# mlvlab/UP-NeRF

Measured on AMD Instinct MI355X. Metric: training rays/sec, higher is better.
Workload: dtype f32 (f16x3 emulated: 3 fp16 MFMAs per product, fp32 accumulate); 1 GPU; BASELINE.json configs[1]: Brandenburg Gate shape, 4096 rays/GPU/step, 64 coarse + 128 fine samples, two 8x256 fields + candidate/colour heads + TransientNet + appearance/candidate embeddings (763 images), pose optimisation ON, full step incl. both Adam updates; rays_per_gpu=4096, n_images=763, N_samples=64, N_importance=128, parallelism=dp1, field=f16x3

## Files before the change

include/upnerf_hip.h:

```cpp
#ifndef UPNERF_HIP_H
#define UPNERF_HIP_H

#include <stdint.h>

#ifdef __cplusplus
extern "C" {
#endif

#define UPNERF_ABI_VERSION 11
#define UPNERF_EINVAL (-1)
#define UPNERF_EUNSUP (-2)

#ifndef UPNERF_TILE_ROWS
#define UPNERF_TILE_ROWS 64
#endif
#define UPNERF_X0 64
#define UPNERF_AUXK 80
#define UPNERF_CK 16
#define UPNERF_MAX_D 8

int upnerf_abi_version(void);

int upnerf_pose_rays_fwd(int R, const float* se3, const float* c2w, const float* dirs,
                         float* rays_o, float* rays_d, void* stream);
// ... 246 lines not shown
int upnerf_transient_fwd(const upnerf_transient_args* a, void* stream);
int upnerf_transient_bwd(const upnerf_transient_args* a, const upnerf_transient_grads* g, void* stream);

enum {
  UPNERF_WG_F32 = 0,
  UPNERF_WG_F16_TILE,
  UPNERF_WG_F16_FRAG,
  UPNERF_WG_F24,
  UPNERF_WG_PLANES
};
typedef struct {
  const void* p;
  const void* lo;
  const int32_t* exp;
  int32_t ld, kind;
} upnerf_wgrad_operand;

typedef struct {
  const float* slabs; const float* bslabs;
  float* dW; float* db;
  int32_t N, K, TN, TK, nsplit, ldo, rblocks;
  int32_t n2;
  float* dW2; float* db2;
  int32_t ldo2, pad;
  const float* vslabs; float* dv; float* dbv;
} upnerf_wgrad_pending;

typedef struct {
  int32_t M, N, K;
  int32_t planes;
  upnerf_wgrad_operand A, B;
  const int32_t* expo_a; const int32_t* expo_b;
  float* dW; float* db;
  int32_t ldo;
  int32_t n2;
  float* dW2; float* db2;
  int32_t ldo2, nsplit;
  const float* v; float* dv; float* dbv;
  float* slabs;
} upnerf_wgrad_desc;
long long upnerf_wgrad16_scratch(const upnerf_wgrad_desc* d);
int upnerf_wgrad16(const upnerf_wgrad_desc* d, upnerf_wgrad_pending* pending, void* stream);
int upnerf_wgrad_finish(upnerf_wgrad_pending* pending, void* stream);

int upnerf_vec_wgrad(int M, const float* v, int ldv, int nvec, const float* X, int ldx, int K,
                     float* dw , float* dbv , float* scratch, int nsplit, void* stream);

int upnerf_vec_wgrad_frag16(int M, const float* v, int ldv, int nvec, const uint16_t* X16, const int32_t* xexp, int K, float* dw,
                            float* dbv, float* scratch, int nsplit, void* stream);

int upnerf_ray_sum(int R, int S, const float* X, int C, float* out, void* stream);
int upnerf_ray_geom_bwd(int R, int S, const float* dxyz, const float* z, float* d_o, float* d_d, void* stream);

typedef struct {
  int32_t R, h, C;
  const int64_t* idx;
  const float* all_ray_infos;
  const float* all_directions;
  const float* all_rgbs;
  const float* all_pxl_coords;
  const float* all_inv_depths;
  const float* feat_maps;
  const float* poses;
  float* ray_infos;
  float* directions;
  int64_t* img_idx;
  float* c2w;
  float* rgbs;
  float* feats;
  float* inv_depths;
} upnerf_gather_rays_args;
int upnerf_gather_rays(const upnerf_gather_rays_args* a, void* stream);

int upnerf_embed_bwd(int R, int N, int dim, const int64_t* idx, const float* g, float* out, void* stream);
#define UPNERF_MAX_EMBED_GROUPS 8
typedef struct {
  const float* g;
  float* out;
  int32_t dim;
} upnerf_embed_group;
int upnerf_embed_bwd_grouped(int R, int N, const int64_t* idx, const upnerf_embed_group* groups, int ngroups, void* stream);
typedef struct {
  const float* table;
  float* rows;
  int32_t dim;
} upnerf_embed_rows_group;
int upnerf_embed_fwd_grouped(int R, int N, const int64_t* idx, const upnerf_embed_rows_group* groups, int ngroups, void* stream);


int upnerf_linear(int M, int N, int K, const float* A, int lda, const float* B, int ldb,
                  const float* bias, float* C, int ldc, int act, void* stream);
int upnerf_matvec(int M, int K, const float* A, int lda, const float* x, const float* add, float* y, int trans, void* stream);
int upnerf_zero(float* p, long long n, void* stream);
#define UPNERF_MAX_ADD_PAIRS 8
typedef struct upnerf_add_pair {
  const float* a;
  const float* b;
  float* out;
  int32_t n;
} upnerf_add_pair;
int upnerf_add_pairs(const upnerf_add_pair* pairs, int npairs, void* stream);
int upnerf_matvec_rank1(int M, int K, const float* A, int lda, const float* x, float* y, float* R, int ldr, const float* v,
                        void* stream);

typedef struct {
  int32_t R, F, fine, has_tw;
// ... 797 lines not shown
```

upnerf_amd/_lib.py:

```python
from __future__ import annotations

import ctypes as C
import os

import torch

from .pass_plan import (AUXK, CK, RR_PART_STRIDE, TILE_PART_STRIDE, WG_F16_FRAG, WG_F16_TILE, WG_F24, WG_F32,
                        WG_PLANES, X0)

_HERE = os.path.dirname(os.path.abspath(__file__))
LIB_PATH = os.environ.get("UPNERF_LIB") or os.path.join(_HERE, "libupnerf_hip.so")
MAX_D = 8

_fp = C.c_void_p


class Layout(C.Structure):
    _fields_ = [("W", C.c_int32), ("D", C.c_int32), ("skip", C.c_int32),
                ("w", C.c_int32 * MAX_D), ("b", C.c_int32 * MAX_D),
                ("we", C.c_int32), ("be", C.c_int32), ("wsig", C.c_int32), ("bsig", C.c_int32),
                ("wc1", C.c_int32), ("bc1", C.c_int32), ("wc2", C.c_int32), ("bc2", C.c_int32),
                ("wcsig", C.c_int32), ("bcsig", C.c_int32), ("wr1", C.c_int32), ("br1", C.c_int32),
                ("wr2", C.c_int32), ("br2", C.c_int32), ("total", C.c_int32),
                ("t_w", C.c_int32 * MAX_D), ("t_skipx", C.c_int32), ("t_we", C.c_int32), ("t_head", C.c_int32),
# ... 93 lines not shown

class WgradPending(C.Structure):
    _fields_ = [("slabs", _fp), ("bslabs", _fp), ("dW", _fp), ("db", _fp), ("N", C.c_int32), ("K", C.c_int32), ("TN", C.c_int32),
                ("TK", C.c_int32), ("nsplit", C.c_int32), ("ldo", C.c_int32), ("rblocks", C.c_int32), ("n2", C.c_int32),
                ("dW2", _fp), ("db2", _fp), ("ldo2", C.c_int32), ("pad", C.c_int32), ("vslabs", _fp), ("dv", _fp), ("dbv", _fp)]


class WgradOperand(C.Structure):
    _fields_ = [("p", _fp), ("lo", _fp), ("exp", _fp), ("ld", C.c_int32), ("kind", C.c_int32)]


class WgradDesc(C.Structure):
    _fields_ = [("M", C.c_int32), ("N", C.c_int32), ("K", C.c_int32), ("planes", C.c_int32), ("A", WgradOperand), ("B", WgradOperand),
                ("expo_a", _fp), ("expo_b", _fp), ("dW", _fp), ("db", _fp), ("ldo", C.c_int32), ("n2", C.c_int32), ("dW2", _fp),
                ("db2", _fp), ("ldo2", C.c_int32), ("nsplit", C.c_int32), ("v", _fp), ("dv", _fp), ("dbv", _fp), ("slabs", _fp)]


class WgradGroup(C.Structure):
    _fields_ = [("A", _fp), ("B", _fp), ("dW", _fp), ("db", _fp), ("M", C.c_int32), ("N", C.c_int32), ("K", C.c_int32),
                ("lda", C.c_int32), ("ldb", C.c_int32), ("ldo", C.c_int32)]


MAX_WGRAD_GROUPS = 32


class EmbedGroup(C.Structure):
    _fields_ = [("g", _fp), ("out", _fp), ("dim", C.c_int32)]


class EmbedRowsGroup(C.Structure):
    _fields_ = [("table", _fp), ("rows", _fp), ("dim", C.c_int32)]


MAX_EMBED_GROUPS = 8


class GatherRaysArgs(C.Structure):
    _fields_ = [("R", C.c_int32), ("h", C.c_int32), ("C", C.c_int32), ("idx", _fp),
                ("all_ray_infos", _fp), ("all_directions", _fp), ("all_rgbs", _fp), ("all_pxl_coords", _fp),
                ("all_inv_depths", _fp), ("feat_maps", _fp), ("poses", _fp),
                ("ray_infos", _fp), ("directions", _fp), ("img_idx", _fp), ("c2w", _fp), ("rgbs", _fp), ("feats", _fp),
                ("inv_depths", _fp)]


class Frag16Desc(C.Structure):
    _fields_ = FragDesc._fields_ + [("exp_id", C.c_int32)]


class AddPair(C.Structure):
    _fields_ = [("a", _fp), ("b", _fp), ("out", _fp), ("n", C.c_int32)]


MAX_ADD_PAIRS = 8


class SsimArgs(C.Structure):
    _fields_ = [("N", C.c_int32), ("C", C.c_int32), ("H", C.c_int32), ("W", C.c_int32), ("pred", _fp), ("gt", _fp),
                ("pred_stride", C.c_int64 * 4), ("gt_stride", C.c_int64 * 4), ("ssim", _fp), ("map", _fp)]


class Conv2dArgs(C.Structure):
    _fields_ = [("N", C.c_int32), ("C_in", C.c_int32), ("H", C.c_int32), ("W", C.c_int32), ("C_out", C.c_int32),
                ("k", C.c_int32), ("stride", C.c_int32), ("pad", C.c_int32), ("relu", C.c_int32), ("scale_in", C.c_int32),
                ("x", _fp), ("x_stride", C.c_int64 * 4), ("w", _fp), ("bias", _fp), ("y", _fp)]


class Maxpool2dArgs(C.Structure):
    _fields_ = [("N", C.c_int32), ("C", C.c_int32), ("H", C.c_int32), ("W", C.c_int32), ("x", _fp), ("y", _fp)]


class LpipsDistArgs(C.Structure):
    _fields_ = [("N", C.c_int32), ("C", C.c_int32), ("H", C.c_int32), ("W", C.c_int32), ("accumulate", C.c_int32),
                ("reserved_", C.c_int32), ("feat", _fp), ("w", _fp), ("out", _fp)]


class LpipsScratchArgs(C.Structure):
    _fields_ = [("N", C.c_int32), ("H", C.c_int32), ("W", C.c_int32), ("reserved_", C.c_int32),
                ("act0_elems", C.c_int64), ("act1_elems", C.c_int64), ("part_elems", C.c_int64)]


class VitPatchesArgs(C.Structure):
    _fields_ = [("H", C.c_int32), ("W", C.c_int32), ("stride", C.c_int32), ("u8", C.c_int32), ("image", _fp),
                ("mean", C.c_float * 3), ("std", C.c_float * 3), ("rows", _fp)]


class VitAttentionArgs(C.Structure):
    _fields_ = [("N", C.c_int32), ("heads", C.c_int32), ("head_dim", C.c_int32), ("reserved_", C.c_int32),
                ("q", _fp), ("k", _fp), ("v", _fp), ("ldq", C.c_int64), ("ldk", C.c_int64), ("ldv", C.c_int64),
                ("scale", C.c_float), ("reserved2_", C.c_float), ("out", _fp), ("ldo", C.c_int64)]


class PcaFitArgs(C.Structure):
    _fields_ = [("T", C.c_int32), ("D", C.c_int32), ("x", _fp), ("ldx", C.c_int64), ("mean", _fp), ("gram", _fp)]


class Conv3x3Args(C.Structure):
    _fields_ = [("H", C.c_int32), ("W", C.c_int32), ("C_in", C.c_int32), ("C_out", C.c_int32), ("stride", C.c_int32),
                ("pre_relu", C.c_int32), ("relu", C.c_int32), ("reserved_", C.c_int32), ("x", _fp), ("ldx", C.c_int64), ("w", _fp),
                ("bias", _fp), ("res", _fp), ("ldr", C.c_int64), ("y", _fp), ("ldy", C.c_int64)]


class Upsample2xArgs(C.Structure):
    _fields_ = [("H", C.c_int32), ("W", C.c_int32), ("C", C.c_int32), ("reserved_", C.c_int32), ("x", _fp), ("ldx", C.c_int64),
                ("y", _fp), ("ldy", C.c_int64)]


# ... 284 lines not shown
    _fields_ = [("M", C.c_int32), ("reserved_", C.c_int32), ("points", _fp), ("P", _fp), ("PT", _fp), ("wk_xyz", C.c_float * 10),
                ("sigma", _fp), ("grad", _fp)]


class NormalCompositeArgs(C.Structure):
    _fields_ = [("R", C.c_int32), ("S", C.c_int32), ("grad", _fp), ("w", _fp), ("normal", _fp)]


class VizNormalsArgs(C.Structure):
    _fields_ = [("H", C.c_int32), ("W", C.c_int32), ("n", _fp), ("rot", _fp), ("rgb", _fp)]


class Rng(C.Structure):
    _fields_ = [("seed", C.c_uint64), ("step", C.c_int32), ("row0", C.c_int32), ("row_stride", C.c_int32), ("step_dev", _fp)]


_i, _f, _p = C.c_int, C.c_float, C.c_void_p
_SIGNATURES = {
    "upnerf_abi_version": [],
    "upnerf_pose_rays_fwd": [_i, _p, _p, _p, _p, _p, _p],
    "upnerf_pose_rays_bwd": [_i, _p, _p, _p, _p, _p, _p, _p],
    "upnerf_sample_coarse": [_i, _i, _p, _p, _p, _f, _i, _p, _p],
    "upnerf_uniform_keyed": [_i, _i, C.c_uint64, _i, _p, _i, _i, _i, _p, _p],
    "upnerf_sample_pdf": [_i, _i, _p, _p, _p, _i, _i, _p, _i, _p],
    "upnerf_sort_rows": [_i, _i, _p, _p],
    "upnerf_sample_coarse_keyed": [_i, _i, _p, _p, C.POINTER(Rng), _f, _i, _p, _p],
    "upnerf_resample_sort": [_i, _i, _p, _p, _i, _i, _p, _i, _p, _i, _i, _p, _i, _i, C.POINTER(Rng), _p, _p],
    "upnerf_ray_aux": [_i, _p, _p, C.POINTER(C.c_float), _p, _p, _p],
    "upnerf_field_fwd": [C.POINTER(Layout), C.POINTER(FieldFwdArgs), _p],
    "upnerf_composite_fwd": [C.POINTER(CompositeFwdArgs), _p],
    "upnerf_composite_bwd": [C.POINTER(CompositeBwdArgs), _p],
    "upnerf_field_bwd": [C.POINTER(Layout), C.POINTER(FieldBwdArgs), _p],
    "upnerf_field_fwd_f16x3": [C.POINTER(Layout), C.POINTER(FieldFwdArgs), _p],
    "upnerf_field_bwd_f16x3": [C.POINTER(Layout), C.POINTER(FieldBwdArgs), _p],
    "upnerf_frag16": [_p, _p, _p, C.POINTER(Frag16Desc), _i, C.POINTER(Frag16Desc), _i, _p, _p, _i, _i, _p, _p],
    "upnerf_wgrad": [_i, _p, _i, _i, _p, _i, _i, _p, _i, _p, _p, _i, _p],
    "upnerf_wgrad16_scratch": [C.POINTER(WgradDesc)],
    "upnerf_wgrad16": [C.POINTER(WgradDesc), C.POINTER(WgradPending), _p],
    "upnerf_wgrad_finish": [_p, _p],
    "upnerf_transient_fwd": [C.POINTER(TransientArgs), _p],
    "upnerf_transient_bwd": [C.POINTER(TransientArgs), C.POINTER(TransientGrads), _p],
    "upnerf_wgrad_grouped_scratch": [C.POINTER(WgradGroup), _i, _i],
    "upnerf_wgrad_grouped": [C.POINTER(WgradGroup), _i, _p, _i, _p],
    "upnerf_vec_wgrad": [_i, _p, _i, _i, _p, _i, _i, _p, _p, _p, _i, _p],
    "upnerf_matvec": [_i, _i, _p, _i, _p, _p, _p, _i, _p],
    "upnerf_matvec_rank1": [_i, _i, _p, _i, _p, _p, _p, _i, _p, _p],
    "upnerf_add_pairs": [C.POINTER(AddPair), _i, _p],
    "upnerf_zero": [_p, C.c_longlong, _p],
    "upnerf_vec_wgrad_frag16": [_i, _p, _i, _i, _p, _p, _i, _p, _p, _p, _i, _p],
    "upnerf_ray_sum": [_i, _i, _p, _i, _p, _p],
    "upnerf_ray_part_finish": [_i, _i, _p, _p, _p, _p],
    "upnerf_tile_part_finish": [_i, _i, _p, _p, _p, _p, _p, _p, _p, _p, _p],
    "upnerf_ray_geom_bwd": [_i, _i, _p, _p, _p, _p, _p],
    "upnerf_pack": [_p, C.POINTER(PackDesc), _i, _i, _p],
    "upnerf_gather_rays": [C.POINTER(GatherRaysArgs), _p],
    "upnerf_embed_bwd": [_i, _i, _i, _p, _p, _p, _p],
    "upnerf_embed_bwd_grouped": [_i, _i, _p, C.POINTER(EmbedGroup), _i, _p],
    "upnerf_embed_fwd_grouped": [_i, _i, _p, C.POINTER(EmbedRowsGroup), _i, _p],
    "upnerf_linear": [_i, _i, _i, _p, _i, _p, _i, _p, _p, _i, _i, _p],
    "upnerf_loss_fwd": [C.POINTER(LossArgs), _p, _p, _p, _p],
    "upnerf_loss_bwd": [C.POINTER(LossArgs), _p, C.POINTER(LossGrads), _p],
    "upnerf_frag_copy": [_p, _p, C.POINTER(FragDesc), _i, _p],
    "upnerf_adam": [C.c_int64, _p, _p, _p, _p, _f, _f, _f, _f, _f, _p, _p],
    "upnerf_adam_gather": [_p, _p, _p, _p, _i, _f, _f, _f, _f, _f, _p, _p],
    "upnerf_set_scalars": [_p, _i, C.POINTER(C.c_float), _p],
    "upnerf_scale_exponents": [_p, _i, _p, _p],
    "upnerf_ssim_scratch": [C.POINTER(SsimArgs)],
    "upnerf_ssim": [C.POINTER(SsimArgs), _p, _p],
    "upnerf_conv2d": [C.POINTER(Conv2dArgs), _p],
    "upnerf_maxpool2d": [C.POINTER(Maxpool2dArgs), _p],
    "upnerf_lpips_dist": [C.POINTER(LpipsDistArgs), _p, _p],
    "upnerf_lpips_scratch": [C.POINTER(LpipsScratchArgs)],
    "upnerf_scene_rays": [C.POINTER(SceneRaysArgs), C.POINTER(SceneImage), _p, _p],
    "upnerf_resize_scratch": [C.POINTER(ResizeArgs)],
    "upnerf_resize_linear": [C.POINTER(ResizeArgs), C.POINTER(ResizeMap), _p, _p],
    "upnerf_viz_minmax_scratch": [C.c_longlong],
    "upnerf_viz_minmax": [_p, C.c_longlong, C.c_longlong, _p, _p, _p],
    "upnerf_viz_depth_scratch": [C.POINTER(VizDepthArgs)],
    "upnerf_viz_depth": [C.POINTER(VizDepthArgs), _p, _p],
    "upnerf_viz_pca_scratch": [C.POINTER(VizPcaArgs)],
    "upnerf_viz_pca": [C.POINTER(VizPcaArgs), _p, _p],
    "upnerf_viz_rgb": [C.POINTER(VizRgbArgs), _p],
    "upnerf_path_poses": [C.POINTER(PathPosesArgs), _p],
    "upnerf_path_rays": [C.POINTER(PathRaysArgs), _p],
    "upnerf_grid_columns": [C.POINTER(GridColumnsArgs), _p],
    "upnerf_mtet_scratch": [_i, _i, _i],
    "upnerf_mtet_count": [C.POINTER(MtetArgs), _p, _p, _p],
    "upnerf_mtet_emit": [C.POINTER(MtetArgs), _p, _p],
    "upnerf_occ_words": [_i, _i, _i],
    "upnerf_occ_build_scratch": [_i, _i, _i],
    "upnerf_occ_build": [C.POINTER(OccBuildArgs), _p],
    "upnerf_occ_spans": [C.POINTER(OccSpansArgs), _p],
    "upnerf_occ_compact_scratch": [_i],
    "upnerf_occ_compact": [C.POINTER(OccCompactArgs), _p],
    "upnerf_occ_scatter": [C.POINTER(OccScatterArgs), _p],
    "upnerf_density_grad": [C.POINTER(Layout), C.POINTER(DensityGradArgs), _p],
    "upnerf_normal_composite": [C.POINTER(NormalCompositeArgs), _p],
    "upnerf_viz_normals": [C.POINTER(VizNormalsArgs), _p],
    "upnerf_tsdf_integrate": [C.POINTER(TsdfIntegrateArgs), _p],
    "upnerf_tsdf_surface": [C.POINTER(TsdfSurfaceArgs), _p],
    "upnerf_tsdf_sample": [C.POINTER(TsdfSampleArgs), _p],
    "upnerf_vit_patches": [C.POINTER(VitPatchesArgs), _p],
    "upnerf_vit_embed": [_i, _i, _p, _p, _p, _p],
    "upnerf_layernorm": [_i, _i, _p, _i, _p, _p, _f, _p, _i, _p],
    "upnerf_vit_attention": [C.POINTER(VitAttentionArgs), _p],
    "upnerf_vit_gelu": [_p, C.c_longlong, _p],
    "upnerf_vit_residual": [_p, _p, C.c_longlong, _p],
    "upnerf_pca_fit_scratch": [_i, _i],
    "upnerf_pca_fit": [C.POINTER(PcaFitArgs), _p, _p],
    "upnerf_conv3x3": [C.POINTER(Conv3x3Args), _p],
    "upnerf_upsample2x": [C.POINTER(Upsample2xArgs), _p],
    "upnerf_depth_to_space": [C.POINTER(DepthToSpaceArgs), _p],
    "upnerf_resize_cubic": [C.POINTER(ResizeCubicArgs), _p],
    "upnerf_vit_patches16": [C.POINTER(VitPatches16Args), _p],
    "upnerf_baked_render": [C.POINTER(BakedRenderArgs), _p],
    "upnerf_baked_pack": [C.POINTER(BakedPackArgs), _p],
    "upnerf_baked_sh_render": [C.POINTER(BakedShRenderArgs), _p],
    "upnerf_sh_accumulate": [C.POINTER(ShAccumulateArgs), _p],
    "upnerf_baked_sh_pack": [C.POINTER(BakedShPackArgs), _p],
    "upnerf_brick_table_scratch": [_i, _i, _i],
    "upnerf_brick_table": [C.POINTER(BrickTableArgs), _p],
    "upnerf_brick_gather": [C.POINTER(BrickGatherArgs), _p],
    "upnerf_brick_scatter": [C.POINTER(BrickScatterArgs), _p],
    "upnerf_brick_occ": [C.POINTER(BrickOccArgs), _p],
    "upnerf_brick_columns": [C.POINTER(BrickColumnsArgs), _p],
    "upnerf_baked_sparse_render": [C.POINTER(BakedSparseRenderArgs), _p],
    "upnerf_baked_render_bwd": [C.POINTER(BakedRenderBwdArgs), _p],
    "upnerf_baked_project": [C.POINTER(BakedProjectArgs), _p],
    "upnerf_baked_sparse_render_bwd": [C.POINTER(BakedSparseRenderBwdArgs), _p],
    "upnerf_brick_face_sum": [C.POINTER(BrickFaceSumArgs), _p],
    "upnerf_baked_ray_bwd": [C.POINTER(BakedRayBwdArgs), _p],
    "upnerf_baked_tv_blocks": [_i, _i, _i, _i],
    "upnerf_baked_tv": [C.POINTER(BakedTvArgs), _p],
    "upnerf_baked_upsample": [C.POINTER(BakedUpsampleArgs), _p],
    "upnerf_brick_upsample_mark": [C.POINTER(BrickUpsampleArgs), _p],
    "upnerf_brick_upsample_fill": [C.POINTER(BrickUpsampleArgs), _p],
    "upnerf_env_rays": [C.POINTER(EnvRaysArgs), _p],
    "upnerf_env_seam": [C.POINTER(EnvSeamArgs), _p],
    "upnerf_env_composite": [C.POINTER(EnvCompositeArgs), _p],
    "upnerf_env_composite_bwd": [C.POINTER(EnvCompositeBwdArgs), _p],
    "upnerf_baked_visibility": [C.POINTER(BakedVisibilityArgs), _p],
    "upnerf_brick_face_max": [C.POINTER(BrickFaceSumArgs), _p],
    "upnerf_baked_prune": [C.POINTER(BakedPruneArgs), _p],
}
_LONGLONG = ("upnerf_wgrad16_scratch", "upnerf_mtet_scratch", "upnerf_occ_words", "upnerf_occ_build_scratch",
             "upnerf_occ_compact_scratch", "upnerf_pca_fit_scratch", "upnerf_brick_table_scratch", "upnerf_baked_tv_blocks")
MAX_SCALARS = 96
EXPORTS = tuple(_SIGNATURES)


def _load():
    if not os.path.exists(LIB_PATH):
        raise ImportError(
            f"{LIB_PATH} not found: the HIP extension is not built. Run `python __graft_entry__.py` "
            "(there is no CPU/PyTorch fallback for the render_rays hot path).")
    lib = C.CDLL(LIB_PATH)
    for name, argtypes in _SIGNATURES.items():
        fn = getattr(lib, name, None)
        if fn is None:
            raise ImportError(f"{LIB_PATH} does not export {name}; rebuild it")
        fn.argtypes = argtypes
        fn.restype = C.c_longlong if name in _LONGLONG else C.c_int
    return lib


lib = _load()
ABI_VERSION = 11
if lib.upnerf_abi_version() != ABI_VERSION:
    raise ImportError("libupnerf_hip.so ABI version mismatch; rebuild it")


_PTR_DTYPES = (torch.float32, torch.int64, torch.int32, torch.float16, torch.uint8, torch.float64)


def ptr(t):
    if t is None:
        return None
    if not t.is_cuda:
        raise RuntimeError("libupnerf_hip operates on device memory only (got a CPU tensor)")
    if not t.is_contiguous():
        raise RuntimeError("non-contiguous tensor handed to the HIP path")
    if t.dtype not in _PTR_DTYPES:
        raise TypeError(f"unsupported dtype {t.dtype} handed to the HIP path")
    return t.data_ptr()


def stream():
    return torch.cuda.current_stream().cuda_stream


CALLS = [0]


def check(rc: int, what: str):
    CALLS[0] += 1
    if rc != 0:
        kind = {-1: "invalid argument", -2: "unsupported shape"}.get(rc, f"hipError_t {rc}")
        raise RuntimeError(f"{what} failed: {kind}")
# ... 1 lines not shown
```

upnerf_amd/rendering.py:

```python
from __future__ import annotations

import ctypes as C
import os
from types import SimpleNamespace
from typing import Dict, List, Optional

import torch

from . import _lib, step_scalars, zero_pool
from ._lib import CompositeBwdArgs, CompositeFwdArgs, FieldBwdArgs, FieldFwdArgs, check, lib, ptr, stream
from .ops import (TIMER, WgOp, WgradRun, embed_rows, fanout, hip_linear, linear_kn_view, linear_raw, nsplit_for,
                  vec_wgrad_frag16_into, vec_wgrad_into, wgrad_into, workspace)
from .pass_plan import DTYPES, MAT, PADDED, RAY, RR_TILE, STAGES, VEC, VEC_FRAG, ZEROED, PassPlan, plan_pass, wgrad_schedule

__all__ = ["render_rays", "sample_pdf", "band_weights", "join_rays", "retain_ray_gradient", "ray_gradient"]


def _env_int(name: str, default: int) -> int:
    return int(os.environ.get("UPNERF_" + name, default))


FIELD_MODE = os.environ.get("UPNERF_FIELD_MODE", "f16x3")
WGRAD_STORE = os.environ.get("UPNERF_WGRAD_STORE", "f32")
TILE_PARTIALS = _env_int("TILE_PARTIALS", 1)
WGRAD_CHAIN = _env_int("WGRAD_CHAIN", 1)
VEC_RIDE = _env_int("VEC_RIDE", 1)
FUSE_RESAMPLE = _env_int("FUSE_RESAMPLE", 1)
JOIN_RAYS = _env_int("JOIN_RAYS", 1)
JOIN_HEADS = _env_int("JOIN_HEADS", 1)
FIELD_RR = _env_int("FIELD_RR", 1)
_SWITCHES = ("FIELD_MODE", "WGRAD_STORE", "FIELD_RR", "TILE_PARTIALS", "WGRAD_CHAIN", "JOIN_HEADS", "VEC_RIDE")


def _plan(pk, R: int, S: int, mode: int = 2, use_cand=False, use_rgb=False, rgb_joint=False, train=False) -> PassPlan:
    sw = {k: globals()[k] for k in _SWITCHES}
    return plan_pass(pk.W, pk.W2, pk.D, R, S, mode, bool(use_cand), bool(use_rgb), bool(rgb_joint), bool(train), **sw)


_PK256 = SimpleNamespace(W=256, W2=128, D=8)
_field16_ok = lambda pk, S: _plan(pk, 1, S).use16
_rr_ok = lambda S: S >= 32 and _plan(_PK256, 1, S).rr
_planes = lambda: _plan(_PK256, 1, 32).planes


_LINSPACE: Dict[tuple, torch.Tensor] = {}
_DEBUG_SINK: Optional[dict] = None


def _linspace01(n: int, device) -> torch.Tensor:
    key = (n, str(device))
    t = _LINSPACE.get(key)
    if t is None:
        t = torch.linspace(0, 1, n, dtype=torch.float32).to(device)
        _LINSPACE[key] = t
    return t


def band_weights(L: int, progress: float, c2f) -> List[float]:
    if c2f is None:
        return [1.0] * L
    start, end = c2f
    alpha = (torch.tensor(float(progress), dtype=torch.float32) - start) / (end - start) * L
    k = torch.arange(L, dtype=torch.float32)
    w = (1 - ((alpha - k).clamp(min=0, max=1) * torch.pi).cos()) / 2
    return [float(x) for x in w]

# ... 78 lines not shown
        return tuple(out[k] if out[k] is not None else z0 for k in outs)

    @staticmethod
    def backward(ctx, gE, gG, gsf, gtw, gcd, gsd, grm, gwall, gws, grj):
        cfg, plan, (R, S), sv = ctx.cfg, ctx.plan, ctx.dims, ctx.saved
        pk, L = cfg.packer, cfg.packer.L
        W, W2, D, M = pk.W, pk.W2, pk.D, plan.M
        dev, st = sv["z"].device, stream()
        joint, want_feat = cfg.mode <= 1, cfg.mode != 2

        def g(t, ok=True):
            return t.contiguous() if (ok and t is not None and t.numel() > 0) else None
        gE, gsf = g(gE, want_feat), g(gsf, want_feat)
        gG, gtw, gcd, gwall = g(gG, joint), g(gtw, joint), g(gcd, joint), g(gwall, joint)
        gsd, gws, grm, grj = g(gsd), g(gws), g(grm, cfg.use_rgb), g(grj, cfg.rgb_joint)
        bw = _alloc(plan, "cbwd", dev)
        cb = _args(CompositeBwdArgs, {**sv, **bw}, R=R, S=S, W=W, mode=cfg.mode, has_rgb=int(cfg.use_rgb), g_E_s=ptr(gE),
                   g_G_c=ptr(gG), g_sum_sfeat=ptr(gsf), g_t_weight=ptr(gtw), g_c_depth=ptr(gcd), g_s_depth=ptr(gsd),
                   g_rgb_map=ptr(grm), g_w_all=ptr(gwall), g_w_s=ptr(gws), g_rgb_joint_map=ptr(grj))
        check(TIMER.run("composite_bwd", lambda: lib.upnerf_composite_bwd(C.byref(cb), st), units=M),
              "upnerf_composite_bwd")
        need_dxyz, P = bool(ctx.needs_input_grad[0] or ctx.needs_input_grad[1]), sv["P"]
        PT = None if plan.use16 else pk.frag_t_hip(P)
        bw.update(_alloc(plan, "fbwd", dev))
        dxyz = _empty(M, 3, device=dev) if need_dxyz else None
        bw.update(_alloc(plan, "part", dev))
        rg = bw["gz_rg"] if plan.joined and not plan.rg16 else None
        gz_r1, gz_g1 = (rg[:, :W2], rg[:, W2:]) if rg is not None else (bw["gz_r1"], bw["gz_g1"])
        dptr = lambda t: None if t is None else t.data_ptr()
        dpre_s, dpre_c, dpre_rgb = bw["dpre_s"], bw["dpre_c"], bw["dpre_rgb"]
        w_feat = (sv["w_sj"] if joint else sv["w_s"]) if gE is not None else None
        fb = _args(FieldBwdArgs, {**sv, **bw}, R=R, S=S, use_cand=int(cfg.use_cand), use_rgb=int(cfg.use_rgb),
                   need_dxyz=int(need_dxyz), PT=ptr(PT), w_feat_s=ptr(w_feat), w_cj=ptr(sv["w_cj"]) if gG is not None else None,
                   g_E_s=ptr(gE), g_G_c=ptr(gG), gmax=ptr(sv["mx32"][16:]), gz_g1=dptr(gz_g1), gz_r1=dptr(gz_r1),
                   gz_rg_ld=W if rg is not None else 0, dpre_sig_s=ptr(dpre_s), dpre_sig_c=ptr(dpre_c), dxyz=ptr(dxyz),
                   planes=plan.planes, tile_rows=plan.tile_rows, tile_part=ptr(bw["ray_part" if plan.rr else "tile_part"]),
                   rows_capacity=plan.rows_capacity)
        bwd_fn = lib.upnerf_field_bwd_f16x3 if plan.use16 else lib.upnerf_field_bwd
        check(TIMER.run("field_bwd", lambda: bwd_fn(C.byref(L), C.byref(fb), st), units=M), "upnerf_field_bwd")
        if _DEBUG_SINK is not None:
            deq = lambda k16, kexp: dequant16(bw[k16][None], bw[kexp][None], frag=True)[0, :M]
            rgf = deq("gz_rg16", "gzrgexp") if plan.rg16 else None
            _DEBUG_SINK.update(
                d_sigma_s=bw["d_sigma_s"], d_sigma_c=bw["d_sigma_c"], d_rgb=bw["d_rgb"],
                gz_h=dequant16(bw["gz16"][:D], bw["gzexp"][:D], frag=plan.rr)[:, :M] if plan.store16 else bw["gz_h"],
                gz_e=dequant16(bw["gz16"][D:], bw["gzexp"][D:], frag=True)[0, :M] if plan.rr else bw["gz_e"],
                gz_g1=rgf[:, W2:] if plan.rg16 else gz_g1, gz_r1=rgf[:, :W2] if plan.rg16 else gz_r1,
                gz_g2=deq("gz_g2_16", "gzg2exp") if plan.g2f else bw["gz_g2"],
                dpre_s=dpre_s, dpre_c=dpre_c, dpre_rgb=dpre_rgb, dxyz=dxyz)
            ctx.bwd_buffers = bw
        dP = zero_pool.zeros(L.total, dev) if ctx.needs_input_grad[5] else None
        d_c_rows = d_a_rows = d_o = d_d = None
        side_c, side_a = pk.block["wc1"].part("c"), pk.block["wr1"].part("a")
        if dP is not None:
            sched = wgrad_schedule(plan, pk.offsets, pk.skip, cfg.use_cand, cfg.use_rgb)
            at = lambda off: None if off is None else dP.data_ptr() + 4 * off
            e32 = torch.empty(32, device=dev, dtype=torch.int32)
            check(lib.upnerf_scale_exponents(ptr(sv["mx32"]), 32, ptr(e32), st), "upnerf_scale_exponents")
            run = WgradRun(dev, chained=WGRAD_CHAIN)
            held = {**sv, **bw}

            def op(name, l=None) -> WgOp:
                o = plan.operands[name]
                i = o.at if l is None else l
                pick = lambda k: None if k is None else held[k] if i is None else held[k][i]
                return WgOp(pick(o.data), o.ld, o.kind, pick(o.exp), pick(o.lo))

            def mat(r):
                head = {} if r.ride is None else dict(v=held[r.ride.v], dv=at(r.ride.dW), dbv=at(r.ride.db))
                run.wgrad(M, op(*r.A), r.N, op(*r.B), r.K, e32.data_ptr() + 4 * (16 + r.ea), e32.data_ptr() + 4 * r.eb, dW=at(r.dW),
                          ldo=r.ldo, db=at(r.db), n2=r.n2, dW2=at(r.dW2), ldo2=r.ldo2, db2=at(r.db2), planes=plan.planes, **head)

            def vec(r):
                v, X = held[r.v], op(*r.B)
                vec_wgrad_into(M, v, v.stride(0), r.N, X.t, X.ld, r.K, at(r.dW), at(r.db), dev)

            def vec_frag(r):
                v, X = held[r.v], op(*r.B)
                vec_wgrad_frag16_into(M, v, v.stride(0), r.N, X.t, X.exp, r.K, at(r.dW), at(r.db), dev)

            def ray(r):
                wgrad_into(R, bw[r.A[0]], r.N, r.N, sv[r.B[0]], r.K, r.K, at(r.dW), r.ldo, None, dev)
            execute = {MAT: mat, VEC: vec, VEC_FRAG: vec_frag, RAY: ray}

            def launch(segment):
                for r in segment:
                    execute[r.kind](r)
            launch(sched.trunk)
        bw.update(_alloc(plan, "sums", dev))
        rs_c, rs_r = bw["rs_c"], bw["rs_r"]
        if plan.partials == "tile":
            tgt = [at(o) for r in sched.part for o in ((r.dW, r.db) if r else (None, None))] if dP is not None else [None] * 4
            check(lib.upnerf_tile_part_finish(R, S, ptr(bw["tile_part"]), ptr(rs_c), ptr(rs_r), *tgt,
                                              ptr(workspace("tile_part", 128 * 520, dev)) if dP is not None else None, st),
                  "upnerf_tile_part_finish")
        elif plan.partials == "ray":
            check(lib.upnerf_ray_part_finish(R, S, ptr(bw["ray_part"]), ptr(rs_c), ptr(rs_r), st), "upnerf_ray_part_finish")
        if cfg.use_cand:
            if plan.partials == "none":
                check(lib.upnerf_ray_sum(R, S, ptr(gz_g1), W2, ptr(rs_c), st), "upnerf_ray_sum")
            if dP is not None:
                launch(sched.cand)
            if ctx.needs_input_grad[3]:
                d_c_rows = linear_kn_view(rs_c, P, L.wc1 + side_c.col0, pk.block["wc1"].ld, side_c.cols)
        if cfg.use_rgb:
            if plan.partials == "none":
                check(lib.upnerf_ray_sum(R, S, ptr(gz_r1), W2, ptr(rs_r), st), "upnerf_ray_sum")
            if dP is not None:
                launch(sched.rgb)
            if ctx.has_a and ctx.needs_input_grad[4]:
                d_a_rows = linear_kn_view(rs_r, P, L.wr1 + side_a.col0, pk.block["wr1"].ld, side_a.cols)
        if dP is not None:
            run.finish()
        if need_dxyz:
            d_o, d_d = _empty(R, 3, device=dev), _empty(R, 3, device=dev)
            check(lib.upnerf_ray_geom_bwd(R, S, ptr(dxyz), ptr(sv["z"]), ptr(d_o), ptr(d_d), st), "upnerf_ray_geom_bwd")
        ctx.saved = None
        return d_o, d_d, None, d_c_rows, d_a_rows, dP, None


def dequant16(t16: torch.Tensor, texp: torch.Tensor, frag: bool = False) -> torch.Tensor:
    D, M, W = t16.shape
    if frag:
        t = t16.view(D, M // 32, W // 16, 2, 32, 2, 4)
        rows = t.permute(0, 1, 4, 2, 5, 3, 6).reshape(D, M, W)
        scale = torch.ldexp(torch.ones((), device=t16.device), -texp.float()).repeat_interleave(32, dim=1)[:, :M]
        return rows.float() * scale[:, :, None]
    scale = torch.ldexp(torch.ones((), device=t16.device), -texp.float()).repeat_interleave(64, dim=1)[:, :M]
    return t16.float() * scale[:, :, None]


def quant16_frag(rows: torch.Tensor, texp: torch.Tensor) -> torch.Tensor:
    M, W = rows.shape
    x = (rows * torch.ldexp(torch.ones((), device=rows.device), texp.float()).repeat_interleave(32)[:, None]).to(torch.float16)
    return x.view(M // 32, 32, W // 16, 2, 2, 4).permute(0, 2, 4, 1, 3, 5).reshape(M, W).contiguous()


def sample_pdf(z_coarse: torch.Tensor, weights: torch.Tensor, n: int, det: bool, out: torch.Tensor, col0: int,
               u: Optional[torch.Tensor] = None):
    R, S = z_coarse.shape
    if n == 0:
        return
    if det:
        uu, rows = _linspace01(n, z_coarse.device), 1
    else:
        uu = u if u is not None else torch.rand(R, n, device=z_coarse.device)
        uu, rows = uu.contiguous(), R
        if tuple(uu.shape) != (R, n):
            raise ValueError(f"sample_pdf: u has shape {tuple(uu.shape)}, expected {(R, n)}")
    stride = out.shape[1]
    check(lib.upnerf_sample_pdf(R, S, ptr(z_coarse), ptr(weights), ptr(uu), rows, n, out.data_ptr() + 4 * col0, stride,
                                stream()), "upnerf_sample_pdf")


_ZEROS = {}


def _zeros(rows, cols, device):
    key = (rows, cols, device)
    if key not in _ZEROS:
        _ZEROS[key] = torch.zeros(rows, cols, device=device)
    return _ZEROS[key]


class _ProjectFeat(torch.autograd.Function):

    @staticmethod
    def forward(ctx, n, *tensors):
        from ._lib import PackDesc
# ... 316 lines not shown
```

Baseline: 256,100 rays/s.

## Fuse per-ray tail backward (ray wgrads, side dx, geometry grads) into one kernel

Replaces the separate per-ray weight-gradient launches, the candidate/appearance input-gradient linear views and the ray geometry backward with one combined kernel. It stages per-ray sums and inputs in LDS, computes dW partials and dx with fp32 MFMAs, and uses extra workgroups in the same grid for the geometry reduction. A second small kernel then reduces the per-block dW slabs. This cuts launch count and re-reads of the per-ray buffers, at the cost of a slab scratch workspace and a fixed-shape kernel with hard size limits. The new kernel uses fp32 MFMAs rather than the emulated f16 path.

```diff
diff --git a/include/upnerf_hip.h b/include/upnerf_hip.h
--- a/include/upnerf_hip.h
+++ b/include/upnerf_hip.h
@@ -322,6 +322,27 @@
 int upnerf_ray_sum(int R, int S, const float* X, int C, float* out, void* stream);
 int upnerf_ray_geom_bwd(int R, int S, const float* dxyz, const float* z, float* d_o, float* d_d, void* stream);
 
+#define UPNERF_RAY_TAIL_ROWS 64
+typedef struct {
+  const float* rs;
+  const float* x;
+  float* dW;
+  const float* w;
+  float* dx;
+  int32_t kx, ldo, ldw, nout;
+} upnerf_ray_tail_side;
+typedef struct {
+  int32_t R, S, N, pad;
+  upnerf_ray_tail_side cand;
+  upnerf_ray_tail_side rgb;
+  const float* dxyz;
+  const float* z;
+  float* d_o; float* d_d;
+  float* slabs;
+} upnerf_ray_tail_args;
+long long upnerf_ray_tail_scratch(const upnerf_ray_tail_args* a);
+int upnerf_ray_tail(const upnerf_ray_tail_args* a, void* stream);
+
 typedef struct {
   int32_t R, h, C;
   const int64_t* idx;
diff --git a/upnerf_amd/_lib.py b/upnerf_amd/_lib.py
--- a/upnerf_amd/_lib.py
+++ b/upnerf_amd/_lib.py
@@ -169,6 +169,19 @@
 
 
 MAX_ADD_PAIRS = 8
+
+
+class RayTailSide(C.Structure):
+    _fields_ = [("rs", _fp), ("x", _fp), ("dW", _fp), ("w", _fp), ("dx", _fp), ("kx", C.c_int32), ("ldo", C.c_int32),
+                ("ldw", C.c_int32), ("nout", C.c_int32)]
+
+
+class RayTailArgs(C.Structure):
+    _fields_ = [("R", C.c_int32), ("S", C.c_int32), ("N", C.c_int32), ("pad", C.c_int32), ("cand", RayTailSide), ("rgb", RayTailSide),
+                ("dxyz", _fp), ("z", _fp), ("d_o", _fp), ("d_d", _fp), ("slabs", _fp)]
+
+
+RAY_TAIL_ROWS = 64
 
 
 class SsimArgs(C.Structure):
@@ -559,6 +572,8 @@
     "upnerf_ray_part_finish": [_i, _i, _p, _p, _p, _p],
     "upnerf_tile_part_finish": [_i, _i, _p, _p, _p, _p, _p, _p, _p, _p, _p],
     "upnerf_ray_geom_bwd": [_i, _i, _p, _p, _p, _p, _p],
+    "upnerf_ray_tail_scratch": [C.POINTER(RayTailArgs)],
+    "upnerf_ray_tail": [C.POINTER(RayTailArgs), _p],
     "upnerf_pack": [_p, C.POINTER(PackDesc), _i, _i, _p],
     "upnerf_gather_rays": [C.POINTER(GatherRaysArgs), _p],
     "upnerf_embed_bwd": [_i, _i, _i, _p, _p, _p, _p],
@@ -650,7 +665,7 @@
     "upnerf_brick_face_max": [C.POINTER(BrickFaceSumArgs), _p],
     "upnerf_baked_prune": [C.POINTER(BakedPruneArgs), _p],
 }
-_LONGLONG = ("upnerf_wgrad16_scratch", "upnerf_mtet_scratch", "upnerf_occ_words", "upnerf_occ_build_scratch",
+_LONGLONG = ("upnerf_wgrad16_scratch", "upnerf_ray_tail_scratch", "upnerf_mtet_scratch", "upnerf_occ_words", "upnerf_occ_build_scratch",
              "upnerf_occ_compact_scratch", "upnerf_pca_fit_scratch", "upnerf_brick_table_scratch", "upnerf_baked_tv_blocks")
 MAX_SCALARS = 96
 EXPORTS = tuple(_SIGNATURES)
diff --git a/upnerf_amd/csrc/ray_tail.hip b/upnerf_amd/csrc/ray_tail.hip
--- /dev/null
+++ b/upnerf_amd/csrc/ray_tail.hip
@@ -0,0 +1,224 @@
+#include "common.cuh"
+
+namespace {
+
+constexpr int RT = UPNERF_RAY_TAIL_ROWS;
+constexpr int RT_NMAX = 128;
+constexpr int RT_LDR = RT_NMAX + 4;
+constexpr int RT_KXMAX = 96;
+constexpr int RT_LDX = RT_KXMAX + 4;
+constexpr int RT_GEO = 4;
+
+static_assert((RT * RT_LDR + RT * RT_LDX) * 4 <= 64 * 1024, "the staged rows must fit the 64 KB a workgroup may hold");
+static_assert(UPNERF_CK <= 32 && UPNERF_AUXK <= RT_KXMAX, "per-ray inputs wider than the tiles below");
+
+template <int KT, int OT>
+__device__ __forceinline__ void side_pass(const upnerf_ray_tail_side& s, int R, int N, int r0, float* __restrict__ rs_s,
+                                          float* __restrict__ x_s, float* __restrict__ slab) {
+  static_assert(2 * OT <= NTHREADS / 64, "one output tile of dx per wave");
+  const int tid = threadIdx.x, lane = tid & 63, wave = tid >> 6;
+  const int li = lane & 31, hh = lane >> 5;
+  const int kx = s.kx;
+  const int rt = wave & 1, ct = wave >> 1;
+  const bool has_dx = s.dx != nullptr && ct < OT && 32 * ct < s.nout;
+  const int col = 32 * ct + li;
+  float wreg[RT_NMAX / 2];
+  if (has_dx) {
+    const bool cin = col < s.nout;
+    const int cc = cin ? col : 0;
+#pragma unroll
+    for (int j = 0; j < RT_NMAX / 2; ++j) {
+      const int k = 8 * (j >> 2) + 4 * hh + (j & 3);
+      const bool in = cin && k < N;
+      wreg[j] = s.w[(size_t)(k < N ? k : 0) * s.ldw + cc];
+      if (!in) wreg[j] = 0.0f;
+    }
+  }
+  const int n4 = N >> 2;
+  for (int idx = tid; idx < RT * n4; idx += NTHREADS) {
+    const int row = idx / n4, c4 = idx - row * n4;
+    const int r = r0 + row;
+    f32x4 v = {0.f, 0.f, 0.f, 0.f};
+    if (r < R) v = *(const f32x4*)&s.rs[(size_t)r * N + 4 * c4];
+    *(f32x4*)&rs_s[row * RT_LDR + 4 * c4] = v;
+  }
+  if (s.dW) {
+    for (int idx = tid; idx < RT * (8 * KT); idx += NTHREADS) {
+      const int row = idx / (8 * KT), c4 = idx - row * (8 * KT);
+      const int r = r0 + row;
+      f32x4 v = {0.f, 0.f, 0.f, 0.f};
+      if (r < R && 4 * c4 < kx) v = *(const f32x4*)&s.x[(size_t)r * kx + 4 * c4];
+      *(f32x4*)&x_s[row * RT_LDX + 4 * c4] = v;
+    }
+  }
+  __syncthreads();
+  if (s.dW && 32 * wave < N) {
+    f32x16 acc[KT];
+#pragma unroll
+    for (int kt = 0; kt < KT; ++kt)
+#pragma unroll
+      for (int r = 0; r < 16; ++r) acc[kt][r] = 0.0f;
+    const float* as = rs_s + hh * RT_LDR + 32 * wave + li;
+    const float* bs = x_s + hh * RT_LDX + li;
+#pragma unroll 4
+    for (int m = 0; m < RT; m += 2) {
+      const float a = as[m * RT_LDR];
+#pragma unroll
+      for (int kt = 0; kt < KT; ++kt)
+        acc[kt] = __builtin_amdgcn_mfma_f32_32x32x2f32(a, bs[m * RT_LDX + 32 * kt], acc[kt], 0, 0, 0);
+    }
+#pragma unroll
+    for (int kt = 0; kt < KT; ++kt) {
+      const int k = 32 * kt + li;
+      if (k < kx) {
+#pragma unroll
+        for (int r = 0; r < 16; ++r) {
+          const int n = 32 * wave + (r & 3) + 8 * (r >> 2) + 4 * hh;
+          slab[n * kx + k] = acc[kt][r];
+        }
+      }
+    }
+  }
+  if (has_dx) {
+    f32x16 acc;
+#pragma unroll
+    for (int r = 0; r < 16; ++r) acc[r] = 0.0f;
+    const float* as = rs_s + (32 * rt + li) * RT_LDR + 4 * hh;
+#pragma unroll
+    for (int t = 0; t < RT_NMAX / 8; ++t) {
+      if (8 * t < N) {
+        const f32x4 a = *(const f32x4*)&as[8 * t];
+#pragma unroll
+        for (int q = 0; q < 4; ++q) acc = __builtin_amdgcn_mfma_f32_32x32x2f32(a[q], wreg[4 * t + q], acc, 0, 0, 0);
+      }
+    }
+    if (col < s.nout) {
+#pragma unroll
+      for (int r = 0; r < 16; ++r) {
+        const int row = r0 + 32 * rt + (r & 3) + 8 * (r >> 2) + 4 * hh;
+        if (row < R) s.dx[(size_t)row * s.nout + col] = acc[r] + 0.0f;
+      }
+    }
+  }
+}
+
+__device__ __forceinline__ int slab_floats(const upnerf_ray_tail_side& s, int N) { return (s.rs && s.dW) ? N * s.kx : 0; }
+
+__global__ __launch_bounds__(NTHREADS) void ray_tail_kernel(upnerf_ray_tail_args a, int nrow) {
+  __shared__ __attribute__((aligned(16))) float rs_s[RT * RT_LDR];
+  __shared__ __attribute__((aligned(16))) float x_s[RT * RT_LDX];
+  if ((int)blockIdx.x >= nrow) {
+    const int wave = threadIdx.x >> 6, lane = threadIdx.x & 63;
+    const int rbase = (((int)blockIdx.x - nrow) * 4 + wave) * RT_GEO;
+    if (rbase >= a.R) return;
+    const int S = a.S;
+    float so[RT_GEO][3], sd[RT_GEO][3];
+#pragma unroll
+    for (int j = 0; j < RT_GEO; ++j)
+#pragma unroll
+      for (int n = 0; n < 3; ++n) so[j][n] = sd[j][n] = 0.f;
+    for (int i = lane; i < S; i += 64) {
+#pragma clang fp contract(off)
+      float zz[RT_GEO], g[RT_GEO][3];
+#pragma unroll
+      for (int j = 0; j < RT_GEO; ++j) {
+        const int r = rbase + j < a.R ? rbase + j : a.R - 1;
+        const size_t m = (size_t)r * S + i;
+        zz[j] = a.z[m];
+#pragma unroll
+        for (int n = 0; n < 3; ++n) g[j][n] = a.dxyz[m * 3 + n];
+      }
+#pragma unroll
+      for (int j = 0; j < RT_GEO; ++j)
+#pragma unroll
+        for (int n = 0; n < 3; ++n) {
+          so[j][n] += g[j][n];
+          sd[j][n] += zz[j] * g[j][n];
+        }
+    }
+#pragma unroll
+    for (int j = 0; j < RT_GEO; ++j) {
+      const int r = rbase + j;
+#pragma unroll
+      for (int n = 0; n < 3; ++n) {
+        const float u = wave_sum(so[j][n]), v = wave_sum(sd[j][n]);
+        if (lane == 0 && r < a.R) {
+          a.d_o[r * 3 + n] = u;
+          a.d_d[r * 3 + n] = v;
+        }
+      }
+    }
+    return;
+  }
+  const int r0 = blockIdx.x * RT;
+  const int nc = slab_floats(a.cand, a.N), nr = slab_floats(a.rgb, a.N);
+  float* slab = a.slabs + (size_t)blockIdx.x * (nc + nr);
+  if (a.cand.rs) side_pass<1, 1>(a.cand, a.R, a.N, r0, rs_s, x_s, slab);
+  if (a.cand.rs && a.rgb.rs) __syncthreads();
+  if (a.rgb.rs) side_pass<3, 2>(a.rgb, a.R, a.N, r0, rs_s, x_s, slab + nc);
+}
+
+__global__ __launch_bounds__(NTHREADS) void ray_tail_reduce_kernel(upnerf_ray_tail_args a, int nrow) {
+  const int nc = slab_floats(a.cand, a.N), nr = slab_floats(a.rgb, a.N);
+  const int e = blockIdx.x * NTHREADS + threadIdx.x;
+  if (e >= nc + nr) return;
+  const size_t stride = (size_t)(nc + nr);
+  const float* src = a.slabs + e;
+  float p0 = 0.f, p1 = 0.f, p2 = 0.f, p3 = 0.f;
+  int b = 0;
+  for (; b + 4 <= nrow; b += 4) {
+    p0 += src[(size_t)b * stride];
+    p1 += src[(size_t)(b + 1) * stride];
+    p2 += src[(size_t)(b + 2) * stride];
+    p3 += src[(size_t)(b + 3) * stride];
+  }
+  for (; b < nrow; ++b) p0 += src[(size_t)b * stride];
+  const upnerf_ray_tail_side& s = e < nc ? a.cand : a.rgb;
+  const int q = e < nc ? e : e - nc;
+  const int n = q / s.kx, k = q - n * s.kx;
+  s.dW[(size_t)n * s.ldo + k] = (p0 + p1) + (p2 + p3);
+}
+
+bool side_ok(const upnerf_ray_tail_side& s, int kxmax, int outmax) {
+  if (!s.rs) return true;
+  if (s.dW && (!s.x || s.kx <= 0 || (s.kx & 3) || s.kx > kxmax || s.ldo < s.kx)) return false;
+  if (s.dx && (!s.w || s.nout <= 0 || s.nout > outmax || s.ldw < s.nout)) return false;
+  return true;
+}
+
+int rows_blocks(int R) { return (R + RT - 1) / RT; }
+
+}
+
+extern "C" long long upnerf_ray_tail_scratch(const upnerf_ray_tail_args* a) {
+  if (!a || a->R <= 0 || a->N <= 0 || a->N > RT_NMAX || (a->N & 31)) return UPNERF_EINVAL;
+  if (!side_ok(a->cand, 32, 32) || !side_ok(a->rgb, RT_KXMAX, 64)) return UPNERF_EINVAL;
+  long long per = 0;
+  if (a->cand.rs && a->cand.dW) per += (long long)a->N * a->cand.kx;
+  if (a->rgb.rs && a->rgb.dW) per += (long long)a->N * a->rgb.kx;
+  return per * rows_blocks(a->R);
+}
+
+extern "C" int upnerf_ray_tail(const upnerf_ray_tail_args* a, void* stream) {
+  if (!a || a->R <= 0) return UPNERF_EINVAL;
+  const bool sides = a->cand.rs || a->rgb.rs;
+  if (sides && (a->N <= 0 || a->N > RT_NMAX || (a->N & 31))) return UPNERF_EINVAL;
+  if (!side_ok(a->cand, 32, 32) || !side_ok(a->rgb, RT_KXMAX, 64)) return UPNERF_EINVAL;
+  if (a->dxyz && (a->S <= 0 || !a->z || !a->d_o || !a->d_d)) return UPNERF_EINVAL;
+  const bool wants_dw = (a->cand.rs && a->cand.dW) || (a->rgb.rs && a->rgb.dW);
+  if (wants_dw && !a->slabs) return UPNERF_EINVAL;
+  upnerf_ray_tail_args k = *a;
+  if (k.cand.rs && !k.cand.dW && !k.cand.dx) k.cand.rs = nullptr;
+  if (k.rgb.rs && !k.rgb.dW && !k.rgb.dx) k.rgb.rs = nullptr;
+  const int nrow = (k.cand.rs || k.rgb.rs) ? rows_blocks(k.R) : 0;
+  const int ngeo = k.dxyz ? (k.R + 4 * RT_GEO - 1) / (4 * RT_GEO) : 0;
+  if (nrow + ngeo == 0) return 0;
+  hipStream_t st = (hipStream_t)stream;
+  hipLaunchKernelGGL(ray_tail_kernel, dim3(nrow + ngeo), dim3(NTHREADS), 0, st, k, nrow);
+  HIP_TRY(hipGetLastError());
+  if (wants_dw) {
+    const int total = (k.cand.dW && k.cand.rs ? k.N * k.cand.kx : 0) + (k.rgb.dW && k.rgb.rs ? k.N * k.rgb.kx : 0);
+    hipLaunchKernelGGL(ray_tail_reduce_kernel, dim3((total + NTHREADS - 1) / NTHREADS), dim3(NTHREADS), 0, st, k, nrow);
+  }
+  return (int)hipGetLastError();
+}
diff --git a/upnerf_amd/rendering.py b/upnerf_amd/rendering.py
--- a/upnerf_amd/rendering.py
+++ b/upnerf_amd/rendering.py
@@ -9,9 +9,9 @@
 
 from . import _lib, step_scalars, zero_pool
 from ._lib import CompositeBwdArgs, CompositeFwdArgs, FieldBwdArgs, FieldFwdArgs, check, lib, ptr, stream
-from .ops import (TIMER, WgOp, WgradRun, embed_rows, fanout, hip_linear, linear_kn_view, linear_raw, nsplit_for,
-                  vec_wgrad_frag16_into, vec_wgrad_into, wgrad_into, workspace)
-from .pass_plan import DTYPES, MAT, PADDED, RAY, RR_TILE, STAGES, VEC, VEC_FRAG, ZEROED, PassPlan, plan_pass, wgrad_schedule
+from .ops import (TIMER, WgOp, WgradRun, embed_rows, fanout, hip_linear, linear_raw, nsplit_for, vec_wgrad_frag16_into,
+                  vec_wgrad_into, workspace)
+from .pass_plan import AUXK, CK, DTYPES, MAT, PADDED, RAY, RR_TILE, STAGES, VEC, VEC_FRAG, ZEROED, PassPlan, plan_pass, wgrad_schedule
 
 __all__ = ["render_rays", "sample_pdf", "band_weights", "join_rays", "retain_ray_gradient", "ray_gradient"]
 
@@ -196,6 +196,7 @@
         dP = zero_pool.zeros(L.total, dev) if ctx.needs_input_grad[5] else None
         d_c_rows = d_a_rows = d_o = d_d = None
         side_c, side_a = pk.block["wc1"].part("c"), pk.block["wr1"].part("a")
+        ray_recs = {}
         if dP is not None:
             sched = wgrad_schedule(plan, pk.offsets, pk.skip, cfg.use_cand, cfg.use_rgb)
             at = lambda off: None if off is None else dP.data_ptr() + 4 * off
@@ -224,7 +225,7 @@
                 vec_wgrad_frag16_into(M, v, v.stride(0), r.N, X.t, X.exp, r.K, at(r.dW), at(r.db), dev)
 
             def ray(r):
-                wgrad_into(R, bw[r.A[0]], r.N, r.N, sv[r.B[0]], r.K, r.K, at(r.dW), r.ldo, None, dev)
+                ray_recs[r.A[0]] = r
             execute = {MAT: mat, VEC: vec, VEC_FRAG: vec_frag, RAY: ray}
 
             def launch(segment):
@@ -246,19 +247,32 @@
             if dP is not None:
                 launch(sched.cand)
             if ctx.needs_input_grad[3]:
-                d_c_rows = linear_kn_view(rs_c, P, L.wc1 + side_c.col0, pk.block["wc1"].ld, side_c.cols)
+                d_c_rows = _empty(R, side_c.cols, device=dev)
         if cfg.use_rgb:
             if plan.partials == "none":
                 check(lib.upnerf_ray_sum(R, S, ptr(gz_r1), W2, ptr(rs_r), st), "upnerf_ray_sum")
             if dP is not None:
                 launch(sched.rgb)
             if ctx.has_a and ctx.needs_input_grad[4]:
-                d_a_rows = linear_kn_view(rs_r, P, L.wr1 + side_a.col0, pk.block["wr1"].ld, side_a.cols)
+                d_a_rows = _empty(R, side_a.cols, device=dev)
         if dP is not None:
             run.finish()
         if need_dxyz:
             d_o, d_d = _empty(R, 3, device=dev), _empty(R, 3, device=dev)
-            check(lib.upnerf_ray_geom_bwd(R, S, ptr(dxyz), ptr(sv["z"]), ptr(d_o), ptr(d_d), st), "upnerf_ray_geom_bwd")
+
+        def side(rs, x, kx, rec, block, part, dx):
+            return _lib.RayTailSide(rs=ptr(rs), x=ptr(x), dW=at(rec.dW) if rec else None, w=P.data_ptr() + 4 * (getattr(L, block) + part.col0),
+                                    dx=ptr(dx), kx=kx, ldo=rec.ldo if rec else 0, ldw=pk.block[block].ld, nout=part.cols)
+        tail = _lib.RayTailArgs(R=R, S=S, N=W2, dxyz=ptr(dxyz), z=ptr(sv["z"]), d_o=ptr(d_o), d_d=ptr(d_d))
+        if cfg.use_cand:
+            tail.cand = side(rs_c, sv["c_rows"], CK, ray_recs.get("rs_c"), "wc1", side_c, d_c_rows)
+        if cfg.use_rgb:
+            tail.rgb = side(rs_r, sv["aux"], AUXK, ray_recs.get("rs_r"), "wr1", side_a, d_a_rows)
+        n = lib.upnerf_ray_tail_scratch(C.byref(tail))
+        if n < 0:
+            check(n, "upnerf_ray_tail_scratch")
+        tail.slabs = ptr(workspace("ray_tail", n, dev)) if n else None
+        check(TIMER.run("ray_tail", lambda: lib.upnerf_ray_tail(C.byref(tail), st), units=R), "upnerf_ray_tail")
         ctx.saved = None
         return d_o, d_d, None, d_c_rows, d_a_rows, dP, None
 
```

Result: no change. 256,000 rays/s (-0.0%).
